# Baverne/VAE-CYCLEGAN-Implementation

Measured on AMD Instinct MI355X. Metric: train images/sec (256x256 VAE-CycleGAN step), higher is better.
Workload: dtype f32; 1 GPU; cyclevaegan unpaired, 3x256x256 synthetic summer<->winter, per-GPU batch 8, latent 64 (BASELINE.json configs[3]/[4]); per_gpu_batch=8, global_batch=8, image_size=256, latent_dim=64, parallelism=dp1, init=random (reference init statistics)

## Files before the change

### vae-cyclegan-implementation_amd/csrc/conv_slab.hip

```cpp
#include "vcg_common.h"

typedef unsigned int sl_u32x4 __attribute__((ext_vector_type(4)));
#define SL_OOB 0x80000000u

struct SlabP {
  const float* in;
  const void* planes;
  const float* bias;
  float* out;
  double* in_part;
  VcgInTail in_tail;
  int N, H, W, C, Ho, Wo, Cout, cout_log;
  int pad, reflect, act, tap_flip, nchunks, in_nchunk;
  int nbx, nby;
  uint32_t in_bytes, b_bytes, row_stride, tap_stride;
  VcgAmax amax_a, amax_b;
};

__device__ __forceinline__ __amdgpu_buffer_rsrc_t sl_srd(const void* ptr, uint32_t bytes) {
  return __builtin_amdgcn_make_buffer_rsrc((void*)ptr, 0, (int)bytes, 0x00020000);
}

template <int WM, int WN, int KH, int KW>
__global__ __launch_bounds__(256, 2) void k_conv_slab(SlabP p) {
  static_assert(WM * WN == 4, "four waves");
  constexpr int BM = 64 * WM, BN = 32 * WN, PR = BM / 16, SH = PR + KH - 1, SW = 16 + KW - 1, SPX = SH * SW, NTAP = KH * KW;
  constexpr int AQ = (SPX * 8 + 255) / 256;
  constexpr int CPR = 4 * VCG_NP;
  constexpr int BQ = (BN * CPR + 255) / 256;
  __shared__ __attribute__((aligned(16))) unsigned char As[VCG_NP][SPX * 64];
  __shared__ __attribute__((aligned(16))) unsigned char Bs[2][VCG_NP][BN * 64];
  const int tid = threadIdx.x, lane = tid & 63, wid = tid >> 6;
  const int wm = wid / WN, wn = wid % WN, l31 = lane & 31, lh = lane >> 5;
  float sA, invA, sB, invB;
  vcg_scale_of(vcg_amax_bits(p.amax_a), p.amax_a.shift, sA, invA);
  vcg_scale_of(vcg_amax_bits(p.amax_b), p.amax_b.shift, sB, invB);
  const float oscale = sA * sB;

  int blk = blockIdx.x;
  const int n = blk / (p.nbx * p.nby);
  blk -= n * p.nbx * p.nby;
  const int by = blk / p.nbx, bx = blk - by * p.nbx;
  const int oy0 = by * PR, ox0 = bx * 16;
  const int n0 = blockIdx.y * BN;

  const __amdgpu_buffer_rsrc_t ra = sl_srd(p.in, p.in_bytes), rb = sl_srd(p.planes, p.b_bytes);

  uint32_t goff[AQ], soff[AQ];
#pragma unroll
  for (int a = 0; a < AQ; ++a) {
    const int idx = tid + 256 * a;
    const int spx = idx >> 3, q = idx & 7;
    const int sy = spx / SW, sx = spx - sy * SW;
    int iy = oy0 + sy - p.pad, ix = ox0 + sx - p.pad;
    bool ok = spx < SPX;
    if (p.reflect) {
      ok = ok && iy >= -p.pad && iy <= p.H - 1 + p.pad && ix >= -p.pad && ix <= p.W - 1 + p.pad;
      iy = reflect_idx(iy, p.H);
      ix = reflect_idx(ix, p.W);
    } else {
      ok = ok && iy >= 0 && iy < p.H && ix >= 0 && ix < p.W;
    }
    goff[a] = ok ? (uint32_t)((((n * p.H + iy) * p.W + ix) * p.C + q * 4) * 4) : SL_OOB;
    soff[a] = spx < SPX ? (uint32_t)(spx * 64 + (((q >> 1) ^ ((spx >> 2) & 3)) << 4) + ((q & 1) << 3)) : SL_OOB;
  }
  uint32_t boff[BQ], bsoff[BQ];
  int bpc[BQ];
#pragma unroll
  for (int j = 0; j < BQ; ++j) {
    const int idx = tid + 256 * j;
    const int row = idx / CPR, r12 = idx - row * CPR, pc = r12 >> 2, q = r12 & 3;
    const bool ok = row < BN;
    boff[j] = ok ? (uint32_t)(n0 + row) * p.row_stride + (uint32_t)(r12 * 16) : SL_OOB;
    bsoff[j] = ok ? (uint32_t)(row * 64 + ((q ^ ((row >> 2) & 3)) << 4)) : SL_OOB;
    bpc[j] = pc;
  }

  f32x16 acc[2], lo[2];
#pragma unroll
  for (int i = 0; i < 2; ++i)
#pragma unroll
    for (int e = 0; e < 16; ++e) acc[i][e] = lo[i][e] = 0.f;

  int rbase[2];
#pragma unroll
  for (int i = 0; i < 2; ++i) {
    const int m = wm * 64 + i * 32 + l31;
    rbase[i] = (m >> 4) * SW + (m & 15);
  }
  const int brow = wn * 32 + l31;
  const uint32_t fb = (uint32_t)(brow * 64);
  const int sb = (brow >> 2) & 3;

  constexpr int PD = NTAP % 3 == 0 ? 3 : NTAP;
  sl_u32x4 vb[PD][BQ];
  const int total = p.nchunks * NTAP;
  auto load_b = [&](sl_u32x4 (&dst)[BQ], int step) {
    const int chunk = step / NTAP, tap = step - chunk * NTAP;
    const uint32_t t = (uint32_t)(p.tap_flip ? NTAP - 1 - tap : tap);
    const uint32_t o = t * p.tap_stride + (uint32_t)chunk * (uint32_t)VCG_PBYTES;
#pragma unroll
    for (int j = 0; j < BQ; ++j) dst[j] = __builtin_amdgcn_raw_buffer_load_b128(rb, (int)(boff[j] != SL_OOB ? boff[j] + o : SL_OOB), 0, 0);
  };
  auto store_b = [&](const sl_u32x4 (&src)[BQ], int buf) {
#pragma unroll
    for (int j = 0; j < BQ; ++j)
      if (bsoff[j] != SL_OOB) *reinterpret_cast<sl_u32x4*>(&Bs[buf][bpc[j]][bsoff[j]]) = src[j];
  };
#pragma unroll
  for (int k = 0; k < PD; ++k)
    if (k < total) load_b(vb[k], k);

  int s = 0;
  for (int chunk = 0; chunk < p.nchunks; ++chunk) {
    {
      float4 va[AQ];
#pragma unroll
      for (int a = 0; a < AQ; ++a) {
        const sl_u32x4 v = __builtin_amdgcn_raw_buffer_load_b128(ra, (int)(goff[a] != SL_OOB ? goff[a] + (uint32_t)chunk * 128u : SL_OOB), 0, 0);
        va[a] = make_float4(__uint_as_float(v.x), __uint_as_float(v.y), __uint_as_float(v.z), __uint_as_float(v.w));
      }
      if (chunk > 0) __syncthreads();
#pragma unroll
      for (int a = 0; a < AQ; ++a) {
        if (soff[a] == SL_OOB) continue;
        uint2 h, l;
        split4h(va[a], invA, h, l);
        *reinterpret_cast<uint2*>(&As[0][soff[a]]) = h;
        *reinterpret_cast<uint2*>(&As[1][soff[a]]) = l;
      }
      if (chunk == 0) {
        store_b(vb[0], 0);
        if (PD < total) load_b(vb[0], PD);
      }
      __syncthreads();
    }
#pragma unroll
    for (int tap = 0; tap < NTAP; ++tap, ++s) {
      const int buf = s & 1;
      const int kh = tap / KW, kw = tap - kh * KW;
      uint32_t fa[2];
      int sa[2];
#pragma unroll
      for (int i = 0; i < 2; ++i) {
        const int r = rbase[i] + kh * SW + kw;
        fa[i] = (uint32_t)(r * 64);
        sa[i] = (r >> 2) & 3;
      }
#pragma unroll
      for (int k2 = 0; k2 < 2; ++k2) {
        f16x8 a[VCG_NP][2], b[VCG_NP];
#pragma unroll
        for (int pc = 0; pc < VCG_NP; ++pc) {
#pragma unroll
          for (int i = 0; i < 2; ++i) a[pc][i] = *reinterpret_cast<const f16x8*>(&As[pc][fa[i] + (((2 * k2 + lh) ^ sa[i]) << 4)]);
          b[pc] = *reinterpret_cast<const f16x8*>(&Bs[buf][pc][fb + (((2 * k2 + lh) ^ sb) << 4)]);
        }
#pragma unroll
        for (int i = 0; i < 2; ++i) {
          f32x16 c = lo[i];
          c = VCG_MFMA(a[1][i], b[0], c);
          c = VCG_MFMA(a[0][i], b[1], c);
          lo[i] = c;
          acc[i] = VCG_MFMA(a[0][i], b[0], acc[i]);
        }
      }
      if (s + 1 < total) {
        constexpr int slot = 0;
        (void)slot;
        const int nslot = (tap + 1) % PD;
#pragma unroll
        for (int k = 0; k < PD; ++k)
          if (k == nslot) {
            store_b(vb[k], buf ^ 1);
            if (s + 1 + PD < total) load_b(vb[k], s + 1 + PD);
          }
      }
      __syncthreads();
    }
  }

  double* const red = reinterpret_cast<double*>(&As[0][0]);
  const int cl = wn * 32 + l31, co = n0 + cl;
  const bool cv = co < p.Cout;
  const float bv = (cv && p.bias && co < p.cout_log) ? p.bias[co] : 0.f;
  double s1 = 0.0, s2 = 0.0;
#pragma unroll
  for (int i = 0; i < 2; ++i) {
#pragma unroll
    for (int e = 0; e < 16; ++e) {
      const int row = (e & 3) + 8 * (e >> 2) + 4 * lh;
      const int m = wm * 64 + i * 32 + row;
      const int oy = oy0 + (m >> 4), ox = ox0 + (m & 15);
      const float v = act_apply((acc[i][e] + lo[i][e]) * oscale + bv, p.act);
      if (cv && oy < p.Ho && ox < p.Wo) p.out[(((size_t)n * p.Ho + oy) * p.Wo + ox) * p.Cout + co] = v;
      if (p.in_part) {
        s1 += (double)v;
        s2 += (double)v * (double)v;
      }
    }
  }
  if (p.in_part) {
    s1 += __shfl_xor(s1, 32);
    s2 += __shfl_xor(s2, 32);
    if (lh == 0) {
      red[(wm * BN + cl) * 2] = s1;
      red[(wm * BN + cl) * 2 + 1] = s2;
    }
    __syncthreads();
    if (tid < BN && n0 + tid < p.Cout) {
      double t1 = 0.0, t2 = 0.0;
#pragma unroll
      for (int w = 0; w < WM; ++w) {
        t1 += red[(w * BN + tid) * 2];
        t2 += red[(w * BN + tid) * 2 + 1];
      }
      double* o = p.in_part + (((size_t)n * p.in_nchunk + blk) * p.Cout + n0 + tid) * 2;
      vcg_store_sc1(o, t1);
      vcg_store_sc1(o + 1, t2);
    }
    if (p.in_tail.out1) {
      __syncthreads();
      vcg_in_tail_run<0>(p.in_tail, p.in_part, n, n0, BN, p.Cout, p.in_nchunk, p.in_tail.counters + n * gridDim.y + blockIdx.y,
                         (uint32_t)p.in_nchunk, reinterpret_cast<double*>(&As[0][0]));
    }
  }
}

__global__ __launch_bounds__(256) void k_fold_pad_c(const float4* __restrict__ dxp, float4* __restrict__ dx, int N, int H, int W, int C4,
                                                    int reflect) {
  const size_t total = (size_t)N * H * W * C4;
  const int Hp = H + 2, Wp = W + 2;
  for (size_t idx = (size_t)blockIdx.x * blockDim.x + threadIdx.x; idx < total; idx += (size_t)gridDim.x * blockDim.x) {
    const int c = (int)(idx % C4);
    size_t r = idx / C4;
    const int w = (int)(r % W);
    r /= W;
    const int h = (int)(r % H), n = (int)(r / H);
    int us[2], vs[2], nu = 0, nv = 0;
    us[nu++] = h + 1;
    vs[nv++] = w + 1;
    if (reflect) {
      if (h == 1) us[nu++] = 0;
      if (h == H - 2) us[nu++] = H + 1;
      if (w == 1) vs[nv++] = 0;
      if (w == W - 2) vs[nv++] = W + 1;
    }
    float4 s = make_float4(0.f, 0.f, 0.f, 0.f);
    for (int a = 0; a < nu; ++a)
      for (int b = 0; b < nv; ++b) {
        const float4 t = dxp[(((size_t)n * Hp + us[a]) * Wp + vs[b]) * C4 + c];
        s.x += t.x; s.y += t.y; s.z += t.z; s.w += t.w;
      }
    dx[idx] = s;
  }
}

static bool slab_geom_ok(const ConvGeom& g) {
  return g.KH == 3 && g.KW == 3 && g.stride == 1 && g.pad == 1 && g.ups == 1 && g.Hl >= 3 && g.Wl >= 3;
}
bool vcg_slab_fwd_ok(const ConvGeom& g) {
  return slab_geom_ok(g) && g.Cin % 32 == 0 && g.Cin <= 128 && g.Cout % 64 == 0 && g.Cout <= 128 && (long long)g.Ho * g.Wo >= 64 * 64;
}
bool vcg_slab_fwd_stats_ok(const ConvGeom& g) { return vcg_slab_fwd_ok(g) && g.Ho % 8 == 0 && g.Wo % 16 == 0; }
int vcg_slab_fwd_nchunk(const ConvGeom& g) { return (g.Ho / 8) * (g.Wo / 16); }
bool vcg_slab_dgrad_ok(const ConvGeom& g) {
  return slab_geom_ok(g) && g.Cout % 32 == 0 && g.Cout <= 128 && (g.Cin == 32 || g.Cin % 64 == 0) && g.Cin <= 128 &&
         (long long)g.H * g.W >= 64 * 64;
}
size_t vcg_slab_dgrad_workspace(const ConvGeom& g) { return (size_t)g.N * (g.H + 2) * (g.W + 2) * g.Cin * sizeof(float) + 256; }

int vcg_slab_fwd(const ConvGeom& g, const float* x, const void* wft_planes, size_t planes_bytes, const void* w_amax, const float* bias,
                 float* y, double* in_part, const VcgInTail* tail_req, hipStream_t st, uint64_t x_handle) {
  SlabP p = {};
  if (vcg_operand_amax(x, (size_t)g.N * g.H * g.W * g.Cin, x_handle, 0, st, &p.amax_a)) return -2;
  p.amax_b = vcg_amax_stored(w_amax);
  p.in = x; p.planes = wft_planes; p.bias = bias; p.out = y; p.in_part = in_part;
  p.N = g.N; p.H = g.H; p.W = g.W; p.C = g.Cin; p.Ho = g.Ho; p.Wo = g.Wo; p.Cout = g.Cout; p.cout_log = g.cout_log;
  p.pad = 1; p.reflect = g.reflect; p.act = g.act; p.tap_flip = 0; p.nchunks = g.Cin / 32;
  p.nbx = (g.Wo + 15) / 16; p.nby = (g.Ho + 7) / 8;
  p.in_nchunk = p.nbx * p.nby;
  p.in_tail = in_part ? vcg_in_tail_make(tail_req->out1, tail_req->out2, g.N * (g.Cout / 64), tail_req->HW, tail_req->eps) : vcg_in_tail_none();
  const unsigned long long ab = (unsigned long long)g.N * g.H * g.W * g.Cin * 4;
  VCG_CHECK_ARG(ab < (1ull << 31) && planes_bytes < (1ull << 31), "vcg_conv_fwd: tensor extents must stay below 2 GiB");
  p.in_bytes = (uint32_t)ab; p.b_bytes = (uint32_t)planes_bytes;
  p.row_stride = (uint32_t)(9 * (g.Cin / 32) * VCG_PBYTES); p.tap_stride = (uint32_t)((g.Cin / 32) * VCG_PBYTES);
  {
    VcgProfScope prof("k_conv_slab<2, 2, 3, 3>", 2.0 * g.M * (double)g.K * g.Cout, st);
    hipLaunchKernelGGL((k_conv_slab<2, 2, 3, 3>), dim3(g.N * p.nbx * p.nby, g.Cout / 64), dim3(256), 0, st, p);
  }
  VCG_LAUNCH_CHECK("vcg_conv_fwd(slab)");
  if (in_part && !p.in_tail.out1)
    return vcg_in_finalize(in_part, tail_req->out1, tail_req->out2, g.N, tail_req->HW, g.Cout, p.in_nchunk, tail_req->eps, st);
  return 0;
}

int vcg_slab_dgrad(const ConvGeom& g, const float* dy, const void* wfd_planes, size_t planes_bytes, const void* w_amax, float* dx,
                   void* ws, size_t ws_bytes, hipStream_t st, uint64_t dy_handle) {
  VCG_CHECK_ARG(ws && ws_bytes >= vcg_slab_dgrad_workspace(g), "vcg_conv_dgrad(slab): workspace too small");
  SlabP p = {};
  if (vcg_operand_amax(dy, (size_t)g.N * g.Ho * g.Wo * g.Cout, dy_handle, 0, st, &p.amax_a)) return -2;
  p.amax_b = vcg_amax_stored(w_amax);
  p.in = dy; p.planes = wfd_planes; p.bias = nullptr; p.out = (float*)ws; p.in_part = nullptr;
  p.N = g.N; p.H = g.Ho; p.W = g.Wo; p.C = g.Cout; p.Ho = g.H + 2; p.Wo = g.W + 2; p.Cout = g.Cin; p.cout_log = g.Cin;
  p.pad = 2; p.reflect = 0; p.act = VCG_ACT_NONE; p.tap_flip = 1; p.nchunks = g.Cout / 32;
  const bool wide = g.Cin == 32;
  p.nbx = (p.Wo + 15) / 16; p.nby = (p.Ho + (wide ? 15 : 7)) / (wide ? 16 : 8);
  const unsigned long long ab = (unsigned long long)g.N * g.Ho * g.Wo * g.Cout * 4;
  VCG_CHECK_ARG(ab < (1ull << 31) && planes_bytes < (1ull << 31), "vcg_conv_dgrad: tensor extents must stay below 2 GiB");
  p.in_bytes = (uint32_t)ab; p.b_bytes = (uint32_t)planes_bytes;
  p.row_stride = (uint32_t)((g.Cout / 32) * VCG_PBYTES); p.tap_stride = (uint32_t)(g.Cin * (g.Cout / 32) * VCG_PBYTES);
  {
    const double flops = 2.0 * g.N * (double)p.Ho * p.Wo * 9.0 * g.Cout * g.Cin;
    VcgProfScope prof(wide ? "k_conv_slab<4, 1, 3, 3>" : "k_conv_slab<2, 2, 3, 3>", flops, st);
    if (wide) hipLaunchKernelGGL((k_conv_slab<4, 1, 3, 3>), dim3(g.N * p.nbx * p.nby, 1), dim3(256), 0, st, p);
    else hipLaunchKernelGGL((k_conv_slab<2, 2, 3, 3>), dim3(g.N * p.nbx * p.nby, g.Cin / 64), dim3(256), 0, st, p);
  }
  VCG_LAUNCH_CHECK("vcg_conv_dgrad(slab)");
  const size_t total = (size_t)g.N * g.H * g.W * (g.Cin / 4);
  int blocks = (int)((total + 255) / 256);
  if (blocks > 4096) blocks = 4096;
  hipLaunchKernelGGL(k_fold_pad_c, dim3(blocks), dim3(256), 0, st, (const float4*)ws, (float4*)dx, g.N, g.H, g.W, g.Cin / 4, g.reflect);
  VCG_LAUNCH_CHECK("vcg_conv_dgrad(slab fold)");
  return 0;
}

bool vcg_slab_col_ok(int KH, int C) { return KH == 7 && C % 32 == 0 && C <= 128; }
int vcg_slab_col(const float* x, const void* planes, size_t planes_bytes, const void* w_amax, float* P, int N, int H, int W, int C,
                 int Ho, int Wo, int KH, int pad, int reflect, hipStream_t st, uint64_t x_handle) {
  VCG_CHECK_ARG(vcg_slab_col_ok(KH, C), "vcg_conv(kw-fold slab): unsupported KH=%d C=%d", KH, C);
  SlabP p = {};
  if (vcg_operand_amax(x, (size_t)N * H * W * C, x_handle, 0, st, &p.amax_a)) return -2;
  p.amax_b = vcg_amax_stored(w_amax);
  p.in = x; p.planes = planes; p.bias = nullptr; p.out = P; p.in_part = nullptr;
  p.N = N; p.H = H; p.W = W; p.C = C; p.Ho = Ho; p.Wo = Wo; p.Cout = 32; p.cout_log = 32;
  p.pad = pad; p.reflect = reflect; p.act = VCG_ACT_NONE; p.tap_flip = 0; p.nchunks = C / 32;
  p.nbx = (Wo + 15) / 16; p.nby = (Ho + 15) / 16;
  const unsigned long long ab = (unsigned long long)N * H * W * C * 4;
  VCG_CHECK_ARG(ab < (1ull << 31) && planes_bytes < (1ull << 31), "vcg_conv(kw-fold slab): tensor extents must stay below 2 GiB");
  p.in_bytes = (uint32_t)ab; p.b_bytes = (uint32_t)planes_bytes;
  p.row_stride = (uint32_t)(KH * (C / 32) * VCG_PBYTES); p.tap_stride = (uint32_t)((C / 32) * VCG_PBYTES);
  {
    VcgProfScope prof("k_conv_slab<4, 1, 7, 1>", 2.0 * N * (double)Ho * Wo * KH * C * 32, st);
    hipLaunchKernelGGL((k_conv_slab<4, 1, 7, 1>), dim3(N * p.nbx * p.nby, 1), dim3(256), 0, st, p);
  }
  VCG_LAUNCH_CHECK("vcg_conv(kw-fold slab)");
  return 0;
}
```

### vae-cyclegan-implementation_amd/csrc/conv_thin.hip

```cpp
#include "vcg_common.h"

struct ThinP {
  const float* x;
  const float* w;
  const float* bias;
  float* out;
  int N, H, W, C, Ho, Wo, K, pad, reflect, n_out, act;
};

#define TT 16
#define CC 16

template <int MODE>
__global__ __launch_bounds__(256) void k_conv_thin(ThinP p) {
  extern __shared__ __attribute__((aligned(16))) float4 patch[];
  const int PS = TT + p.K - 1, PP = PS * PS;
  const int tx = threadIdx.x & 15, ty = threadIdx.x >> 4;
  const int ox0 = blockIdx.x * TT, oy0 = blockIdx.y * TT, n = blockIdx.z;
  float acc0 = 0.f, acc1 = 0.f, acc2 = 0.f, acc3 = 0.f;
  const float* xn = p.x + (size_t)n * p.H * p.W * p.C;
  const int KK = p.K * p.K;

  for (int c0 = 0; c0 < p.C; c0 += CC) {
    __syncthreads();
    for (int idx = threadIdx.x; idx < PP * (CC / 4); idx += 256) {
      const int j = idx & (CC / 4 - 1), pos = idx / (CC / 4);
      const int py = pos / PS, px = pos - py * PS;
      int iy = oy0 + py - p.pad, ix = ox0 + px - p.pad;
      float4 v = make_float4(0.f, 0.f, 0.f, 0.f);
      bool ok;
      if (p.reflect) {
        ok = iy > -p.H && iy < 2 * p.H - 1 && ix > -p.W && ix < 2 * p.W - 1 && iy >= -p.pad && ix >= -p.pad &&
             iy <= p.H - 1 + p.pad && ix <= p.W - 1 + p.pad;
        if (ok) { iy = reflect_idx(iy, p.H); ix = reflect_idx(ix, p.W); }
      } else {
        ok = iy >= 0 && iy < p.H && ix >= 0 && ix < p.W;
      }
      if (ok) v = *reinterpret_cast<const float4*>(xn + ((size_t)iy * p.W + ix) * p.C + c0 + j * 4);
      patch[j * PP + pos] = v;
    }
    __syncthreads();
    for (int tap = 0; tap < KK; ++tap) {
      const int ky = tap / p.K, kx = tap - ky * p.K;
      const int pos = (ty + ky) * PS + tx + kx;
#pragma unroll
      for (int j = 0; j < CC / 4; ++j) {
        const float4 v = patch[j * PP + pos];
        const int c = c0 + j * 4;
        if (MODE == 0) {
          const float* wp = p.w + ((size_t)tap * p.C + c) * 4;
          acc0 += v.x * wp[0] + v.y * wp[4] + v.z * wp[8] + v.w * wp[12];
          acc1 += v.x * wp[1] + v.y * wp[5] + v.z * wp[9] + v.w * wp[13];
          acc2 += v.x * wp[2] + v.y * wp[6] + v.z * wp[10] + v.w * wp[14];
        } else {
          const float* wp = p.w + ((size_t)(KK - 1 - tap) * 4) * p.C + c;
          acc0 += v.x * wp[0] + v.y * wp[1] + v.z * wp[2] + v.w * wp[3];
          const float* w1 = wp + p.C;
          acc1 += v.x * w1[0] + v.y * w1[1] + v.z * w1[2] + v.w * w1[3];
          const float* w2 = w1 + p.C;
          acc2 += v.x * w2[0] + v.y * w2[1] + v.z * w2[2] + v.w * w2[3];
        }
      }
    }
  }
  const int oy = oy0 + ty, ox = ox0 + tx;
  if (oy < p.Ho && ox < p.Wo) {
    float4 o = make_float4(acc0, acc1, acc2, acc3);
    if (p.bias) {
      if (p.n_out > 0) o.x += p.bias[0];
      if (p.n_out > 1) o.y += p.bias[1];
      if (p.n_out > 2) o.z += p.bias[2];
    }
    if (p.n_out < 3) o.z = 0.f;
    if (p.n_out < 2) o.y = 0.f;
    o.x = act_apply(o.x, p.act); o.y = act_apply(o.y, p.act); o.z = act_apply(o.z, p.act);
    *reinterpret_cast<float4*>(p.out + (((size_t)n * p.Ho + oy) * p.Wo + ox) * 4) = o;
  }
}

__global__ __launch_bounds__(256) void k_fold_pad(const float4* __restrict__ dxp, float4* __restrict__ dx, int N, int H,
                                                  int W, int pad, int reflect) {
  const size_t total = (size_t)N * H * W;
  const int Hp = H + 2 * pad, Wp = W + 2 * pad;
  for (size_t idx = (size_t)blockIdx.x * blockDim.x + threadIdx.x; idx < total; idx += (size_t)gridDim.x * blockDim.x) {
    const int w = (int)(idx % W);
    const size_t r = idx / W;
    const int h = (int)(r % H), n = (int)(r / H);
    int us[3], vs[3], nu = 0, nv = 0;
    us[nu++] = h + pad;
    vs[nv++] = w + pad;
    if (reflect) {
      if (h >= 1 && h <= pad) us[nu++] = pad - h;
      if (h >= H - 1 - pad && h <= H - 2) us[nu++] = 2 * (H - 1) - h + pad;
      if (w >= 1 && w <= pad) vs[nv++] = pad - w;
      if (w >= W - 1 - pad && w <= W - 2) vs[nv++] = 2 * (W - 1) - w + pad;
    }
    float4 s = make_float4(0.f, 0.f, 0.f, 0.f);
    for (int a = 0; a < nu; ++a)
      for (int b = 0; b < nv; ++b) {
        const float4 t = dxp[((size_t)n * Hp + us[a]) * Wp + vs[b]];
        s.x += t.x; s.y += t.y; s.z += t.z; s.w += t.w;
      }
    dx[idx] = s;
  }
}

bool vcg_thin_fwd_ok(const ConvGeom& g) {
  return g.Cout == 4 && g.stride == 1 && g.ups == 1 && g.KH == g.KW && (g.KH & 1) && g.Cin % CC == 0 &&
         g.pad == g.KH / 2;
}
bool vcg_thin_dgrad_ok(const ConvGeom& g) {
  return g.Cin == 4 && g.stride == 1 && g.ups == 1 && g.KH == g.KW && (g.KH & 1) && g.Cout % CC == 0 &&
         g.pad == g.KH / 2;
}
size_t vcg_thin_dgrad_workspace(const ConvGeom& g) {
  return (size_t)g.N * (g.H + 2 * g.pad) * (g.W + 2 * g.pad) * 4 * sizeof(float) + 256;
}

int vcg_fwd_launch(const ConvGeom& g, const float* x, const float* wf, float* y, hipStream_t st);
bool vcg_slab_col_ok(int KH, int C);
int vcg_slab_col(const float* x, const void* planes, size_t planes_bytes, const void* w_amax, float* P, int N, int H, int W, int C, int Ho, int Wo,
                 int KH, int pad, int reflect, hipStream_t st, uint64_t x_handle);
static size_t fold_planes_floats(int KH, int C) { return vcg_slab_col_ok(KH, C) ? (size_t)KH * C * VCG_PFLOATS : 0; }
__global__ __launch_bounds__(256) void k_fold_planes(const float* __restrict__ wk, unsigned short* __restrict__ bp, int K, VcgAmax amax) {
  float sc, inv;
  vcg_scale_of(vcg_amax_bits(amax), amax.shift, sc, inv);
  const int total = 32 * (K / 4);
  for (int idx = blockIdx.x * blockDim.x + threadIdx.x; idx < total; idx += gridDim.x * blockDim.x) {
    const int n = idx / (K / 4), k0 = (idx - n * (K / 4)) * 4;
    const float4 v = make_float4(wk[(size_t)(k0 + 0) * 32 + n], wk[(size_t)(k0 + 1) * 32 + n], wk[(size_t)(k0 + 2) * 32 + n],
                                 wk[(size_t)(k0 + 3) * 32 + n]);
    uint2 h, l;
    split4h(v, inv, h, l);
    unsigned short* o = bp + ((size_t)n * (K / 32) + k0 / 32) * VCG_PBLK + (k0 & 31);
    *reinterpret_cast<uint2*>(o) = h;
    *reinterpret_cast<uint2*>(o + 32) = l;
  }
}
static int pack_fold_planes(float* wk, int KH, int C, const VcgAmax& amax_w, hipStream_t st) {
  if (!fold_planes_floats(KH, C)) return 0;
  const int K = KH * C;
  hipLaunchKernelGGL(k_fold_planes, dim3((32 * (K / 4) + 255) / 256), dim3(256), 0, st, (const float*)wk,
                     (unsigned short*)(wk + (size_t)K * 32), K, amax_w);
  VCG_LAUNCH_CHECK("vcg_pack_weight(kw-fold planes)");
  return 0;
}

bool vcg_thin_fold_ok(const ConvGeom& g) { return vcg_thin_fwd_ok(g) && g.KW * 4 <= 32 && g.cout_log <= 3; }
size_t vcg_thin_fold_weight_floats(const ConvGeom& g) { return (size_t)g.KH * g.Cin * 32 + fold_planes_floats(g.KH, g.Cin); }
size_t vcg_thin_fold_workspace(const ConvGeom& g) {
  return (size_t)g.N * g.Ho * (g.W + 2 * g.pad) * 32 * sizeof(float) + 256;
}
__global__ __launch_bounds__(256) void k_pack_kwfold(const float* __restrict__ w, float* __restrict__ wk, int C, int cin_log,
                                                     int cout_log, int KH, int KW) {
  const int total = KH * C * 32;
  for (int idx = blockIdx.x * blockDim.x + threadIdx.x; idx < total; idx += gridDim.x * blockDim.x) {
    const int col = idx & 31, row = idx >> 5;
    const int kh = row / C, c = row - kh * C;
    const int kw = col >> 2, co = col & 3;
    float v = 0.f;
    if (kw < KW && co < cout_log && c < cin_log) v = w[(((size_t)co * cin_log + c) * KH + kh) * KW + kw];
    wk[idx] = v;
  }
}
__global__ __launch_bounds__(256) void k_pack_kwfold_dgrad(const float* __restrict__ w, float* __restrict__ wk, int Cout,
                                                           int cin_log, int cout_log, int KH, int KW) {
  const int total = KH * Cout * 32;
  for (int idx = blockIdx.x * blockDim.x + threadIdx.x; idx < total; idx += gridDim.x * blockDim.x) {
    const int col = idx & 31, row = idx >> 5;
    const int kh = row / Cout, co = row - kh * Cout;
    const int kw = col >> 2, ci = col & 3;
    float v = 0.f;
    if (kw < KW && ci < cin_log && co < cout_log) v = w[(((size_t)co * cin_log + ci) * KH + (KH - 1 - kh)) * KW + (KW - 1 - kw)];
    wk[idx] = v;
  }
}
bool vcg_thin_fold_dgrad_ok(const ConvGeom& g) { return vcg_thin_dgrad_ok(g) && g.KW * 4 <= 32 && g.cin_log <= 3; }
size_t vcg_thin_fold_dgrad_weight_floats(const ConvGeom& g) { return (size_t)g.KH * g.Cout * 32 + fold_planes_floats(g.KH, g.Cout); }
int vcg_thin_fold_dgrad_pack(const ConvGeom& g, const float* w_oihw, float* wk, const VcgAmax& amax_w, hipStream_t st) {
  const int total = g.KH * g.Cout * 32;
  hipLaunchKernelGGL(k_pack_kwfold_dgrad, dim3((total + 255) / 256), dim3(256), 0, st, w_oihw, wk, g.Cout, g.cin_log,
                     g.cout_log, g.KH, g.KW);
  VCG_LAUNCH_CHECK("vcg_pack_weight(kw-fold dgrad)");
  return pack_fold_planes(wk, g.KH, g.Cout, amax_w, st);
}
static ConvGeom thin_dgrad_as_fwd(const ConvGeom& g) {
  ConvGeom f = g;
  f.H = g.Ho; f.W = g.Wo; f.Hl = g.Ho; f.Wl = g.Wo; f.Cin = g.Cout; f.cin_log = g.cout_log; f.Cout = 4; f.cout_log = g.cin_log;
  f.pad = 2 * g.pad; f.reflect = 0; f.act = VCG_ACT_NONE;
  f.Ho = g.H + 2 * g.pad; f.Wo = g.W + 2 * g.pad;
  f.M = f.N * f.Ho * f.Wo; f.K = f.KH * f.KW * f.Cin; f.taps = f.KH * f.KW;
  return f;
}
size_t vcg_thin_fold_dgrad_workspace(const ConvGeom& g) {
  const ConvGeom f = thin_dgrad_as_fwd(g);
  return vcg_thin_dgrad_workspace(g) + 256 + vcg_thin_fold_workspace(f);
}

int vcg_thin_fold_pack(const ConvGeom& g, const float* w_oihw, float* wk, const VcgAmax& amax_w, hipStream_t st) {
  const int total = g.KH * g.Cin * 32;
  hipLaunchKernelGGL(k_pack_kwfold, dim3((total + 255) / 256), dim3(256), 0, st, w_oihw, wk, g.Cin, g.cin_log, g.cout_log, g.KH,
                     g.KW);
  VCG_LAUNCH_CHECK("vcg_pack_weight(kw-fold)");
  return pack_fold_planes(wk, g.KH, g.Cin, amax_w, st);
}
__global__ __launch_bounds__(256) void k_kwfold_sum(const float* __restrict__ P, const float* __restrict__ bias,
                                                    float* __restrict__ y, int N, int H, int W, int Wp, int KW, int n_out,
                                                    int act) {
  const size_t total = (size_t)N * H * W;
  for (size_t idx = (size_t)blockIdx.x * blockDim.x + threadIdx.x; idx < total; idx += (size_t)gridDim.x * blockDim.x) {
    const int ow = (int)(idx % W);
    const size_t row = idx / W;
    const float* pr = P + (row * Wp + ow) * 32;
    float4 s = make_float4(0.f, 0.f, 0.f, 0.f);
    for (int kw = 0; kw < KW; ++kw) {
      const float4 v = *reinterpret_cast<const float4*>(pr + (size_t)kw * 32 + kw * 4);
      s.x += v.x; s.y += v.y; s.z += v.z; s.w += v.w;
    }
    if (bias) {
      if (n_out > 0) s.x += bias[0];
      if (n_out > 1) s.y += bias[1];
      if (n_out > 2) s.z += bias[2];
    }
    s.w = 0.f;
    if (n_out < 3) s.z = 0.f;
    if (n_out < 2) s.y = 0.f;
    s.x = act_apply(s.x, act); s.y = act_apply(s.y, act); s.z = act_apply(s.z, act);
    *reinterpret_cast<float4*>(y + idx * 4) = s;
  }
}
int vcg_thin_fold_fwd(const ConvGeom& g, const float* x, const float* wk, const void* w_amax, const float* bias, float* y, void* ws,
                      size_t ws_bytes, hipStream_t st, uint64_t x_handle) {
  VCG_CHECK_ARG(ws && ws_bytes >= vcg_thin_fold_workspace(g), "vcg_conv_fwd: workspace too small for the kw-folded path");
  ConvGeom q = g;
  q.KW = 1; q.Cout = 32; q.cout_log = g.KW * 4; q.act = VCG_ACT_NONE;
  q.Wo = g.W + 2 * g.pad; q.Ho = g.Ho; q.M = g.N * q.Ho * q.Wo; q.taps = g.KH; q.K = g.KH * g.Cin;
  if (fold_planes_floats(g.KH, g.Cin)) {
    if (vcg_slab_col(x, wk + (size_t)g.KH * g.Cin * 32, fold_planes_floats(g.KH, g.Cin) * 4, w_amax, (float*)ws, g.N, g.H, g.W, g.Cin, q.Ho,
                     q.Wo, g.KH, g.pad, g.reflect, st, x_handle))
      return -2;
  } else if (vcg_fwd_launch(q, x, wk, (float*)ws, st)) {
    return -2;
  }
  const size_t total = (size_t)g.N * g.Ho * g.Wo;
  int blocks = (int)((total + 255) / 256);
  if (blocks > 4096) blocks = 4096;
  hipLaunchKernelGGL(k_kwfold_sum, dim3(blocks), dim3(256), 0, st, (const float*)ws, bias, y, g.N, g.Ho, g.Wo, q.Wo, g.KW,
                     g.cout_log < 3 ? g.cout_log : 3, g.act);
  VCG_LAUNCH_CHECK("vcg_conv_fwd(kw-fold sum)");
  return 0;
}

int vcg_thin_fwd(const ConvGeom& g, const float* x, const float* wf, const float* bias, float* y, hipStream_t st) {
  ThinP p;
  p.x = x; p.w = wf; p.bias = bias; p.out = y;
  p.N = g.N; p.H = g.H; p.W = g.W; p.C = g.Cin; p.Ho = g.Ho; p.Wo = g.Wo; p.K = g.KH; p.pad = g.pad;
  p.reflect = g.reflect; p.n_out = g.cout_log < 3 ? g.cout_log : 3; p.act = g.act;
  const int PS = TT + g.KH - 1;
  const size_t lds = (size_t)PS * PS * CC * sizeof(float);
  VCG_CHECK_ARG(lds <= 64 * 1024, "vcg_conv_fwd(thin): kernel %d too large for the LDS patch", g.KH);
  VCG_CHECK_ARG(g.cout_log <= 3, "vcg_conv_fwd(thin): at most 3 logical output channels");
  dim3 grid((g.Wo + TT - 1) / TT, (g.Ho + TT - 1) / TT, g.N);
  hipLaunchKernelGGL(k_conv_thin<0>, grid, dim3(256), lds, st, p);
  VCG_LAUNCH_CHECK("vcg_conv_fwd(thin)");
  return 0;
}

int vcg_thin_fold_dgrad(const ConvGeom& g, const float* dy, const float* wkd, const void* w_amax, float* dx, void* ws, size_t ws_bytes,
                        hipStream_t st, uint64_t dy_handle) {
  VCG_CHECK_ARG(ws && ws_bytes >= vcg_thin_fold_dgrad_workspace(g), "vcg_conv_dgrad(kw-fold): workspace too small");
  const ConvGeom f = thin_dgrad_as_fwd(g);
  float* dxp = (float*)ws;
  char* ws2 = (char*)ws + ((vcg_thin_dgrad_workspace(g) + 255) / 256) * 256;
  if (vcg_thin_fold_fwd(f, dy, wkd, w_amax, nullptr, dxp, ws2, ws_bytes - (size_t)(ws2 - (char*)ws), st, dy_handle)) return -2;
  size_t total = (size_t)g.N * g.H * g.W;
  int blocks = (int)((total + 255) / 256);
  if (blocks > 2048) blocks = 2048;
  hipLaunchKernelGGL(k_fold_pad, dim3(blocks), dim3(256), 0, st, (const float4*)dxp, (float4*)dx, g.N, g.H, g.W, g.pad,
                     g.reflect);
  VCG_LAUNCH_CHECK("vcg_conv_dgrad(kw-fold)");
  return 0;
}

int vcg_thin_dgrad(const ConvGeom& g, const float* dy, const float* wf, float* dx, void* ws, size_t ws_bytes,
                   hipStream_t st) {
  VCG_CHECK_ARG(ws && ws_bytes >= vcg_thin_dgrad_workspace(g), "vcg_conv_dgrad(thin): workspace too small");
  VCG_CHECK_ARG(g.cin_log <= 3, "vcg_conv_dgrad(thin): at most 3 logical input channels");
  ThinP p;
  p.x = dy; p.w = wf; p.bias = nullptr; p.out = (float*)ws;
  p.N = g.N; p.H = g.Ho; p.W = g.Wo; p.C = g.Cout; p.K = g.KH;
  p.pad = 2 * g.pad;
  p.Ho = g.H + 2 * g.pad; p.Wo = g.W + 2 * g.pad;
  p.reflect = 0; p.n_out = g.cin_log; p.act = VCG_ACT_NONE;
  const int PS = TT + g.KH - 1;
  const size_t lds = (size_t)PS * PS * CC * sizeof(float);
  VCG_CHECK_ARG(lds <= 64 * 1024, "vcg_conv_dgrad(thin): kernel %d too large for the LDS patch", g.KH);
  dim3 grid((p.Wo + TT - 1) / TT, (p.Ho + TT - 1) / TT, g.N);
  hipLaunchKernelGGL(k_conv_thin<1>, grid, dim3(256), lds, st, p);
  size_t total = (size_t)g.N * g.H * g.W;
  int blocks = (int)((total + 255) / 256);
  if (blocks > 2048) blocks = 2048;
  hipLaunchKernelGGL(k_fold_pad, dim3(blocks), dim3(256), 0, st, (const float4*)ws, (float4*)dx, g.N, g.H, g.W, g.pad,
                     g.reflect);
  VCG_LAUNCH_CHECK("vcg_conv_dgrad(thin)");
  return 0;
}
```

Baseline: 253.8 images/s.

## Fuse kw-fold column sum into the 7x7 thin-output slab conv kernel

Adds a templated tile width and a fused kw-fold mode to the slab conv kernel. The 7x1 column-GEMM results for a 32-wide tile are staged in LDS and summed across the seven kw shifts in-kernel, with bias and activation applied, then written straight to the 4-channel output. This removes the intermediate P workspace write/read and the separate k_kwfold_sum launch. In exchange, overlapping tiles (26 useful of 32 columns) recompute some halo work, and the path can be disabled with an environment variable.

```diff
diff --git a/vae-cyclegan-implementation_amd/csrc/conv_slab.hip b/vae-cyclegan-implementation_amd/csrc/conv_slab.hip
--- a/vae-cyclegan-implementation_amd/csrc/conv_slab.hip
+++ b/vae-cyclegan-implementation_amd/csrc/conv_slab.hip
@@ -15,16 +15,21 @@
   int nbx, nby;
   uint32_t in_bytes, b_bytes, row_stride, tap_stride;
   VcgAmax amax_a, amax_b;
+  int fold_nout;
 };
 
 __device__ __forceinline__ __amdgpu_buffer_rsrc_t sl_srd(const void* ptr, uint32_t bytes) {
   return __builtin_amdgcn_make_buffer_rsrc((void*)ptr, 0, (int)bytes, 0x00020000);
 }
 
-template <int WM, int WN, int KH, int KW>
+template <int WM, int WN, int KH, int KW, int TW = 16, int FKW = 0>
 __global__ __launch_bounds__(256, 2) void k_conv_slab(SlabP p) {
   static_assert(WM * WN == 4, "four waves");
-  constexpr int BM = 64 * WM, BN = 32 * WN, PR = BM / 16, SH = PR + KH - 1, SW = 16 + KW - 1, SPX = SH * SW, NTAP = KH * KW;
+  static_assert(FKW == 0 || (KW == 1 && WN == 1 && FKW * 4 <= 32 && TW >= 2 * FKW), "fused kw-fold sum: one 32-column tile of (kw, co)");
+  constexpr int BM = 64 * WM, BN = 32 * WN, PR = BM / TW, SH = PR + KH - 1, SW = TW + KW - 1, SPX = SH * SW, NTAP = KH * KW;
+  constexpr int OWT = TW - (FKW > 0 ? FKW - 1 : 0);
+  constexpr int PST = 36;
+  static_assert(FKW == 0 || BM * PST * 4 <= VCG_NP * SPX * 64, "the P tile reuses the slab's LDS");
   constexpr int AQ = (SPX * 8 + 255) / 256;
   constexpr int CPR = 4 * VCG_NP;
   constexpr int BQ = (BN * CPR + 255) / 256;
@@ -41,7 +46,7 @@
   const int n = blk / (p.nbx * p.nby);
   blk -= n * p.nbx * p.nby;
   const int by = blk / p.nbx, bx = blk - by * p.nbx;
-  const int oy0 = by * PR, ox0 = bx * 16;
+  const int oy0 = by * PR, ox0 = bx * OWT;
   const int n0 = blockIdx.y * BN;
 
   const __amdgpu_buffer_rsrc_t ra = sl_srd(p.in, p.in_bytes), rb = sl_srd(p.planes, p.b_bytes);
@@ -86,7 +91,7 @@
 #pragma unroll
   for (int i = 0; i < 2; ++i) {
     const int m = wm * 64 + i * 32 + l31;
-    rbase[i] = (m >> 4) * SW + (m & 15);
+    rbase[i] = (m / TW) * SW + (m % TW);
   }
   const int brow = wn * 32 + l31;
   const uint32_t fb = (uint32_t)(brow * 64);
@@ -183,6 +188,41 @@
   double* const red = reinterpret_cast<double*>(&As[0][0]);
   const int cl = wn * 32 + l31, co = n0 + cl;
   const bool cv = co < p.Cout;
+  if constexpr (FKW > 0) {
+    float* const pt = reinterpret_cast<float*>(&As[0][0]);
+#pragma unroll
+    for (int i = 0; i < 2; ++i) {
+#pragma unroll
+      for (int e = 0; e < 16; ++e) {
+        const int m = wm * 64 + i * 32 + (e & 3) + 8 * (e >> 2) + 4 * lh;
+        pt[m * PST + cl] = (acc[i][e] + lo[i][e]) * oscale + 0.f;
+      }
+    }
+    __syncthreads();
+    for (int idx = tid; idx < PR * OWT; idx += 256) {
+      const int r = idx / OWT, c = idx - r * OWT;
+      const int oy = oy0 + r, ox = ox0 + c;
+      if (oy >= p.Ho || ox >= p.Wo) continue;
+      const float* pr = pt + (r * TW + c) * PST;
+      float4 s = make_float4(0.f, 0.f, 0.f, 0.f);
+#pragma unroll
+      for (int kw = 0; kw < FKW; ++kw) {
+        const float4 v = *reinterpret_cast<const float4*>(pr + kw * PST + kw * 4);
+        s.x += v.x; s.y += v.y; s.z += v.z; s.w += v.w;
+      }
+      if (p.bias) {
+        if (p.fold_nout > 0) s.x += p.bias[0];
+        if (p.fold_nout > 1) s.y += p.bias[1];
+        if (p.fold_nout > 2) s.z += p.bias[2];
+      }
+      s.w = 0.f;
+      if (p.fold_nout < 3) s.z = 0.f;
+      if (p.fold_nout < 2) s.y = 0.f;
+      s.x = act_apply(s.x, p.act); s.y = act_apply(s.y, p.act); s.z = act_apply(s.z, p.act);
+      *reinterpret_cast<float4*>(p.out + (((size_t)n * p.Ho + oy) * p.Wo + ox) * 4) = s;
+    }
+    return;
+  }
   const float bv = (cv && p.bias && co < p.cout_log) ? p.bias[co] : 0.f;
   double s1 = 0.0, s2 = 0.0;
 #pragma unroll
@@ -191,7 +231,7 @@
     for (int e = 0; e < 16; ++e) {
       const int row = (e & 3) + 8 * (e >> 2) + 4 * lh;
       const int m = wm * 64 + i * 32 + row;
-      const int oy = oy0 + (m >> 4), ox = ox0 + (m & 15);
+      const int oy = oy0 + m / TW, ox = ox0 + m % TW;
       const float v = act_apply((acc[i][e] + lo[i][e]) * oscale + bv, p.act);
       if (cv && oy < p.Ho && ox < p.Wo) p.out[(((size_t)n * p.Ho + oy) * p.Wo + ox) * p.Cout + co] = v;
       if (p.in_part) {
@@ -326,20 +366,26 @@
 }
 
 bool vcg_slab_col_ok(int KH, int C) { return KH == 7 && C % 32 == 0 && C <= 128; }
-int vcg_slab_col(const float* x, const void* planes, size_t planes_bytes, const void* w_amax, float* P, int N, int H, int W, int C,
-                 int Ho, int Wo, int KH, int pad, int reflect, hipStream_t st, uint64_t x_handle) {
+static int slab_col_params(SlabP& p, const float* x, const void* planes, size_t planes_bytes, const void* w_amax, int N, int H, int W, int C,
+                           int KH, int pad, int reflect, hipStream_t st, uint64_t x_handle) {
   VCG_CHECK_ARG(vcg_slab_col_ok(KH, C), "vcg_conv(kw-fold slab): unsupported KH=%d C=%d", KH, C);
-  SlabP p = {};
   if (vcg_operand_amax(x, (size_t)N * H * W * C, x_handle, 0, st, &p.amax_a)) return -2;
   p.amax_b = vcg_amax_stored(w_amax);
-  p.in = x; p.planes = planes; p.bias = nullptr; p.out = P; p.in_part = nullptr;
-  p.N = N; p.H = H; p.W = W; p.C = C; p.Ho = Ho; p.Wo = Wo; p.Cout = 32; p.cout_log = 32;
-  p.pad = pad; p.reflect = reflect; p.act = VCG_ACT_NONE; p.tap_flip = 0; p.nchunks = C / 32;
-  p.nbx = (Wo + 15) / 16; p.nby = (Ho + 15) / 16;
+  p.in = x; p.planes = planes; p.in_part = nullptr;
+  p.N = N; p.H = H; p.W = W; p.C = C; p.Cout = 32; p.cout_log = 32;
+  p.pad = pad; p.reflect = reflect; p.tap_flip = 0; p.nchunks = C / 32;
   const unsigned long long ab = (unsigned long long)N * H * W * C * 4;
   VCG_CHECK_ARG(ab < (1ull << 31) && planes_bytes < (1ull << 31), "vcg_conv(kw-fold slab): tensor extents must stay below 2 GiB");
   p.in_bytes = (uint32_t)ab; p.b_bytes = (uint32_t)planes_bytes;
   p.row_stride = (uint32_t)(KH * (C / 32) * VCG_PBYTES); p.tap_stride = (uint32_t)((C / 32) * VCG_PBYTES);
+  return 0;
+}
+int vcg_slab_col(const float* x, const void* planes, size_t planes_bytes, const void* w_amax, float* P, int N, int H, int W, int C,
+                 int Ho, int Wo, int KH, int pad, int reflect, hipStream_t st, uint64_t x_handle) {
+  SlabP p = {};
+  if (slab_col_params(p, x, planes, planes_bytes, w_amax, N, H, W, C, KH, pad, reflect, st, x_handle)) return -2;
+  p.bias = nullptr; p.out = P; p.Ho = Ho; p.Wo = Wo; p.act = VCG_ACT_NONE;
+  p.nbx = (Wo + 15) / 16; p.nby = (Ho + 15) / 16;
   {
     VcgProfScope prof("k_conv_slab<4, 1, 7, 1>", 2.0 * N * (double)Ho * Wo * KH * C * 32, st);
     hipLaunchKernelGGL((k_conv_slab<4, 1, 7, 1>), dim3(N * p.nbx * p.nby, 1), dim3(256), 0, st, p);
@@ -347,3 +393,19 @@
   VCG_LAUNCH_CHECK("vcg_conv(kw-fold slab)");
   return 0;
 }
+bool vcg_slab_col_fold_ok(int KH, int KW, int C) { return vcg_slab_col_ok(KH, C) && KW == 7; }
+int vcg_slab_col_fold(const float* x, const void* planes, size_t planes_bytes, const void* w_amax, const float* bias, float* y, int N, int H,
+                      int W, int C, int Ho, int Wo, int KH, int KW, int pad, int reflect, int act, int n_out, hipStream_t st,
+                      uint64_t x_handle) {
+  VCG_CHECK_ARG(vcg_slab_col_fold_ok(KH, KW, C), "vcg_conv(fused kw-fold slab): unsupported KH=%d KW=%d C=%d", KH, KW, C);
+  SlabP p = {};
+  if (slab_col_params(p, x, planes, planes_bytes, w_amax, N, H, W, C, KH, pad, reflect, st, x_handle)) return -2;
+  p.bias = bias; p.out = y; p.Ho = Ho; p.Wo = Wo; p.act = act; p.fold_nout = n_out;
+  p.nbx = (Wo + 25) / 26; p.nby = (Ho + 7) / 8;
+  {
+    VcgProfScope prof("k_conv_slab<4, 1, 7, 1>", 2.0 * N * (double)Ho * (p.nbx * 32) * KH * C * 32, st);
+    hipLaunchKernelGGL((k_conv_slab<4, 1, 7, 1, 32, 7>), dim3(N * p.nbx * p.nby, 1), dim3(256), 0, st, p);
+  }
+  VCG_LAUNCH_CHECK("vcg_conv(fused kw-fold slab)");
+  return 0;
+}
diff --git a/vae-cyclegan-implementation_amd/csrc/conv_thin.hip b/vae-cyclegan-implementation_amd/csrc/conv_thin.hip
--- a/vae-cyclegan-implementation_amd/csrc/conv_thin.hip
+++ b/vae-cyclegan-implementation_amd/csrc/conv_thin.hip
@@ -1,3 +1,4 @@
+#include <stdlib.h>
 #include "vcg_common.h"
 
 struct ThinP {
@@ -121,6 +122,10 @@
 bool vcg_slab_col_ok(int KH, int C);
 int vcg_slab_col(const float* x, const void* planes, size_t planes_bytes, const void* w_amax, float* P, int N, int H, int W, int C, int Ho, int Wo,
                  int KH, int pad, int reflect, hipStream_t st, uint64_t x_handle);
+bool vcg_slab_col_fold_ok(int KH, int KW, int C);
+int vcg_slab_col_fold(const float* x, const void* planes, size_t planes_bytes, const void* w_amax, const float* bias, float* y, int N, int H,
+                      int W, int C, int Ho, int Wo, int KH, int KW, int pad, int reflect, int act, int n_out, hipStream_t st, uint64_t x_handle);
+static bool kwfold_fuse_on() { const char* e = getenv("VCG_KWFOLD_FUSE"); return !e || atoi(e) != 0; }
 static size_t fold_planes_floats(int KH, int C) { return vcg_slab_col_ok(KH, C) ? (size_t)KH * C * VCG_PFLOATS : 0; }
 __global__ __launch_bounds__(256) void k_fold_planes(const float* __restrict__ wk, unsigned short* __restrict__ bp, int K, VcgAmax amax) {
   float sc, inv;
@@ -235,6 +240,9 @@
   ConvGeom q = g;
   q.KW = 1; q.Cout = 32; q.cout_log = g.KW * 4; q.act = VCG_ACT_NONE;
   q.Wo = g.W + 2 * g.pad; q.Ho = g.Ho; q.M = g.N * q.Ho * q.Wo; q.taps = g.KH; q.K = g.KH * g.Cin;
+  if (fold_planes_floats(g.KH, g.Cin) && vcg_slab_col_fold_ok(g.KH, g.KW, g.Cin) && kwfold_fuse_on())
+    return vcg_slab_col_fold(x, wk + (size_t)g.KH * g.Cin * 32, fold_planes_floats(g.KH, g.Cin) * 4, w_amax, bias, y, g.N, g.H, g.W, g.Cin, g.Ho,
+                             g.Wo, g.KH, g.KW, g.pad, g.reflect, g.act, g.cout_log < 3 ? g.cout_log : 3, st, x_handle);
   if (fold_planes_floats(g.KH, g.Cin)) {
     if (vcg_slab_col(x, wk + (size_t)g.KH * g.Cin * 32, fold_planes_floats(g.KH, g.Cin) * 4, w_amax, (float*)ws, g.N, g.H, g.W, g.Cin, q.Ho,
                      q.Wo, g.KH, g.pad, g.reflect, st, x_handle))
```

After: 247.7 images/s. -2.4%, worse.
